# ivargr/kmer_mapper

Hardware: AMD Instinct MI355X
Metric: M k-mers mapped/sec (whole node), k=31 150bp reads (higher is better)
Workload: dtype u64

## Files before the change

kmer_mapper_amd/csrc/kmm_radix.hpp:

```cpp
#pragma once
#include <type_traits>
#include "kmm_radix_plan.hpp"

constexpr int RX_NT = 512;
constexpr int RX_KPT = RX_B / RX_NT;
#ifndef RX_LPR2V
#define RX_LPR2V 16
#endif
constexpr int RX_LPR = RX_LPR2V;
constexpr int RX_NG = RX_NT / RX_LPR;
#ifndef RX_RB1
#define RX_RB1 4
#endif
#ifndef RX_RB2
#define RX_RB2 8
#endif
constexpr int RX_SUBCAP = 1024;
#ifndef RX_SUBCAP3V
#define RX_SUBCAP3V 3072
#endif
constexpr int RX_SUBCAP3 = RX_SUBCAP3V;
#ifndef RX_LPR3
#define RX_LPR3 16
#endif
// ... 77 lines not shown
    const uint64_t quo = fastdiv_m31(q, (uint32_t)iv.modulo, iv.magic, &h);
    *coarse = h >> sh;
    return (quo << sh) | (uint64_t)(h & ((1u << sh) - 1u));
}

__device__ __forceinline__ uint2 rx_pair(const uint32_t *s_in, int c0, int n)
{
    const uint2 p = *reinterpret_cast<const uint2 *>(s_in + c0);
    return make_uint2(c0 < n ? p.x : 0u, c0 + 1 < n ? p.y : 0u);
}

template <bool ONEBAR>
__device__ __forceinline__ uint32_t rx_scan256(const uint32_t *s_in, uint32_t *s_out, int n, uint32_t *s_wave, const int tid)
{
    if (ONEBAR) {
    (void)s_wave;
    const int lane = tid & 63;
    const int wave = __builtin_amdgcn_readfirstlane(tid >> 6);
    if (wave < 4) {
        const uint32_t v = tid < n ? s_in[tid] : 0u;
        const uint32_t inc = wave_scan_incl(v);
        uint32_t before = 0;
        for (int x = 0; x < wave; ++x) {
            const uint32_t t = x * 64 + lane < n ? s_in[x * 64 + lane] : 0u;
            before += (uint32_t)__builtin_amdgcn_readlane((int)wave_scan_incl(t), 63);
        }
        if (tid < n)
            s_out[tid] = before + inc - v;
        if (tid == 255)
            s_out[n] = before + inc;
    }
    __syncthreads();
    return s_out[n];
    }
    const int lane = tid & 63, wave = tid >> 6;
    const uint32_t v = tid < n ? s_in[tid] : 0u;
    const uint32_t inc = wave_scan_incl(v);
    if (wave < 4 && lane == 63)
        s_wave[wave] = inc;
    __syncthreads();
    const uint32_t total = s_wave[0] + s_wave[1] + s_wave[2] + s_wave[3];
    if (tid < n) {
        uint32_t base = 0;
        for (int x = 0; x < wave; ++x)
            base += s_wave[x];
        s_out[tid] = base + inc - v;
    }
    if (tid == 0)
        s_out[n] = total;
    __syncthreads();
    return total;
}

template <bool ONEBAR>
__device__ __forceinline__ uint32_t rx_scan512(const uint32_t *s_in, uint32_t *s_out, int n, uint32_t *s_wave, const int tid)
{
    const int lane = tid & 63;
    const int wave = __builtin_amdgcn_readfirstlane(tid >> 6);
    if (ONEBAR) {
    (void)s_wave;
    if (wave < 4) {
        const int c0 = wave * 128 + lane * 2;
        const uint2 p = rx_pair(s_in, c0, n);
        const uint32_t v = p.x + p.y;
        const uint32_t inc = wave_scan_incl(v);
        uint32_t before = 0;
        for (int x = 0; x < wave; ++x) {
            const uint2 t = rx_pair(s_in, x * 128 + lane * 2, n);
            before += (uint32_t)__builtin_amdgcn_readlane((int)wave_scan_incl(t.x + t.y), 63);
        }
        const uint32_t ex = before + inc - v;
        if (c0 < n)
            s_out[c0] = ex;
        if (c0 + 1 < n)
            s_out[c0 + 1] = ex + p.x;
        if (tid == 255)
            s_out[n] = before + inc;
    }
    __syncthreads();
    return s_out[n];
    }
    uint2 p = make_uint2(0u, 0u);
    uint32_t v = 0, inc = 0;
    const int c0 = wave * 128 + lane * 2;
    if (wave < 4) {
        p = rx_pair(s_in, c0, n);
        v = p.x + p.y;
        inc = wave_scan_incl(v);
        if (lane == 63)
            s_wave[wave] = inc;
    }
    __syncthreads();
    const uint32_t total = s_wave[0] + s_wave[1] + s_wave[2] + s_wave[3];
    if (wave < 4) {
        uint32_t base = 0;
        for (int x = 0; x < wave; ++x)
            base += s_wave[x];
        const uint32_t ex = base + inc - v;
        if (c0 < n)
            s_out[c0] = ex;
        if (c0 + 1 < n)
            s_out[c0 + 1] = ex + p.x;
    }
    if (tid == 0)
        s_out[n] = total;
    __syncthreads();
    return total;
}

#ifdef RX_PHASE_TIMERS
#define RX_PT_DECL unsigned long long pt_acc[7] = {0, 0, 0, 0, 0, 0, (unsigned long long)clock64()}
#define RX_PT_ARG , pt_acc
#define RX_PT_ARG2 , pt_acc
#define RX_PT(slot)                                                                                                   \
    do {                                                                                                              \
        if (threadIdx.x == 0) {                                                                                       \
            const unsigned long long pt_now = (unsigned long long)clock64();                                                            \
            pt_acc[slot] += pt_now - pt_acc[6];                                                                       \
            pt_acc[6] = pt_now;                                                                                       \
        }                                                                                                             \
    } while (0)
#define RX_PT_END(iv, base)                                                                                           \
    do {                                                                                                              \
        if (threadIdx.x == 0)                                                                                         \
            for (int pt_i = 0; pt_i < 6; ++pt_i)                                                                      \
                atomicAdd(&(iv).stats[(size_t)(blockIdx.x % KMM_STAT_SHARDS) * KMM_STAT_STRIDE + (base) + pt_i],     \
                          pt_acc[pt_i]);                                                                              \
    } while (0)
#else
#define RX_PT_DECL
#define RX_PT_ARG
#define RX_PT_ARG2 , nullptr
#define RX_PT(slot)
#define RX_PT_END(iv, base)
#endif

__device__ __forceinline__ int rx_tid_now(int wave)
{
    int l;
    asm volatile("v_mbcnt_lo_u32_b32 %0, -1, 0\n\tv_mbcnt_hi_u32_b32 %0, -1, %0" : "=v"(l));
    return (wave << 6) | l;
}

__device__ __forceinline__ uint32_t rx_spare_key()
{
    return (uint32_t)RX_MAXF + 1u + (threadIdx.x & 63);
}

struct RxNoHook {
    __device__ __forceinline__ void operator()() const {}
};

template <int RB, bool ENDBAR, bool ONEBAR, int NT = RX_NT, bool NTSTORE = ONEBAR, typename PrepFn,
          typename MidFn = RxNoHook, int WAVESCAN = 0, bool NOWTID = false, typename PostFn = RxNoHook, int CAPMAX = RX_B>
__device__ __forceinline__ void rx_sort_emit(uint64_t (&q)[RX_B / NT], PrepFn prep, int F, uint64_t *sbuf,
                                             uint32_t *s_cnt, uint32_t *s_base, uint32_t *s_wave,
                                             uint64_t *__restrict__ out, uint16_t *__restrict__ dir_row,
                                             unsigned long long *pt_acc = nullptr, MidFn mid = MidFn(),
                                             int n_slots = RX_B / NT, int wave_s = -1, PostFn post = PostFn(),
                                             uint64_t *probe_out = nullptr, int probe_den = 0, uint32_t cap = RX_B,
                                             unsigned long long *multi_stat = nullptr)
{
    static_assert(CAPMAX <= RX_B && CAPMAX % 2 == 0, "rounds start at 16-byte boundaries of the output");
    constexpr bool ROUNDS = CAPMAX < RX_B;
    auto tid_now = [&]() { return NOWTID ? rx_tid_now(wave_s) : (int)threadIdx.x; };
    constexpr int KPT = RX_B / NT;
    int tid = tid_now();
    (void)pt_acc;
    uint32_t cr[KPT];
#pragma unroll
    for (int h = 0; h < KPT; h += RB) {
        if (h >= n_slots) {
#pragma unroll
            for (int i = 0; i < RB; ++i)
                cr[h + i] = 0xFFFF0000u;
            continue;
        }
        uint32_t ck[RB], rk[RB];
#pragma unroll
        for (int i = 0; i < RB; ++i)
            ck[i] = prep(h + i);
#pragma unroll
        for (int i = 0; i < RB; ++i)
            rk[i] = atomicAdd(&s_cnt[ck[i]], 1u);
#pragma unroll
        for (int i = 0; i < RB; ++i)
            cr[h + i] = (ck[i] << 16) | (rk[i] & 0xFFFFu);
    }
    __syncthreads();
    RX_PT(2);
    mid();
    uint32_t total;
    uint32_t packed = 0;
    const bool by_wave = WAVESCAN == 2 || (WAVESCAN == 1 && F <= 128);
    auto pos_of = [&](int h) {
        const uint32_t key = cr[h] >> 16;
        if (by_wave) {
            const uint32_t pk = (uint32_t)__builtin_amdgcn_ds_bpermute((int)((key >> 1) << 2), (int)packed);
            return (pk & 0xFFFFu) + ((key & 1u) ? pk >> 16 : 0u) + (cr[h] & 0xFFFFu);
        }
        return s_base[key < (uint32_t)F ? key : 0u] + (cr[h] & 0xFFFFu);
    };
    auto place_first = [&]() {
#pragma unroll
        for (int h = 0; h < KPT; ++h) {
            if (h >= n_slots)
                break;
            const uint32_t pos = pos_of(h);
            if ((cr[h] >> 16) < (uint32_t)F && pos < cap)
                sbuf[pos] = q[h];
        }
    };
    if (by_wave) {
        const int lane = tid & 63;
        const uint2 p = rx_pair(s_cnt, lane * 2, F);
        const uint32_t inc = wave_scan_incl(p.x + p.y);
        const uint32_t ex0 = inc - p.x - p.y;
        total = (uint32_t)__builtin_amdgcn_readlane((int)inc, 63);
        if (tid < 64) {
            if (2 * lane <= F)
                dir_row[2 * lane] = (uint16_t)ex0;
            if (2 * lane + 1 <= F)
                dir_row[2 * lane + 1] = (uint16_t)(ex0 + p.x);
            if (lane == 63 && F == 128)
                dir_row[128] = (uint16_t)inc;
        }
        packed = ex0 | (p.x << 16);
        if (ROUNDS && total > cap) {
            place_first();
        } else {
#pragma unroll
        for (int h = 0; h < KPT; ++h) {
            if (h >= n_slots)
                break;
            const uint32_t key = cr[h] >> 16;
            const uint32_t pk = (uint32_t)__builtin_amdgcn_ds_bpermute((int)((key >> 1) << 2), (int)packed);
            const uint32_t pos = (pk & 0xFFFFu) + ((key & 1u) ? pk >> 16 : 0u) + (cr[h] & 0xFFFFu);
            if (key < (uint32_t)F)
                sbuf[pos] = q[h];
        }
        }
    } else {
    tid = tid_now();
    total = F <= 256 ? rx_scan256<ONEBAR>(s_cnt, s_base, F, s_wave, tid) : rx_scan512<ONEBAR>(s_cnt, s_base, F, s_wave, tid);
    tid = tid_now();
    if (tid <= F)
        s_cnt[tid] = 0;
    if (NT == RX_MAXF && F == NT && tid == 0)
        s_cnt[NT] = 0;
    if (tid <= F)
        dir_row[tid] = (uint16_t)s_base[tid];
    if (NT == RX_MAXF && F == NT && tid == 0)
        dir_row[NT] = (uint16_t)s_base[NT];
    if (ROUNDS && total > cap) {
        place_first();
    } else {
#pragma unroll
    for (int h = 0; h < KPT; ++h) {
        if (h >= n_slots)
            break;
        const uint32_t pos = s_base[cr[h] >> 16] + (cr[h] & 0xFFFFu);
        if ((cr[h] >> 16) < (uint32_t)F)
            sbuf[pos] = q[h];
    }
    }
    }
    post();
    __syncthreads();
    RX_PT(3);
    tid = tid_now();
    if (by_wave) {
        if (tid <= F)
            s_cnt[tid] = 0;
        if (NT == RX_MAXF && F == NT && tid == 0)
            s_cnt[NT] = 0;
    }
    const uint4 *s4 = reinterpret_cast<const uint4 *>(sbuf);
    uint4 *o4 = reinterpret_cast<uint4 *>(out);
    const uint32_t n_first = ROUNDS && total > cap ? cap : total;
    for (uint32_t i = tid; i < (n_first + 1) / 2; i += NT) {
        if (NTSTORE) {
            typedef uint32_t u32x4_t __attribute__((ext_vector_type(4)));
            const uint4 v = s4[i];
            const u32x4_t w = {v.x, v.y, v.z, v.w};
            __builtin_nontemporal_store(w, reinterpret_cast<u32x4_t *>(o4) + i);
        } else {
            o4[i] = s4[i];
        }
        if (RX_PROBE_ANY && probe_den > 0 && i % (uint32_t)probe_den == 0u) {
            if (NTSTORE) {
                typedef uint32_t u32x4_t __attribute__((ext_vector_type(4)));
                const uint4 v = s4[i];
                const u32x4_t w = {v.x, v.y, v.z, v.w};
                __builtin_nontemporal_store(w, reinterpret_cast<u32x4_t *>(probe_out) + i / (uint32_t)probe_den);
            } else {
                reinterpret_cast<uint4 *>(probe_out)[i / (uint32_t)probe_den] = s4[i];
            }
        }
    }
    if constexpr (ROUNDS) {
        if (total > cap) {
            for (uint32_t lo = cap; lo < total; lo += cap) {
                __syncthreads();
#pragma unroll
                for (int h = 0; h < KPT; ++h) {
                    if (h >= n_slots)
                        break;
                    const uint32_t pos = pos_of(h) - lo;
                    if ((cr[h] >> 16) < (uint32_t)F && pos < cap)
                        sbuf[pos] = q[h];
                }
                __syncthreads();
                const uint32_t n = total - lo < cap ? total - lo : cap;
                uint4 *o4r = reinterpret_cast<uint4 *>(out + lo);
                for (uint32_t i = tid; i < (n + 1) / 2; i += NT)
                    o4r[i] = s4[i];
            }
            if (multi_stat && tid == 0)
                atomicAdd(multi_stat, 1ull);
        }
    }
    if (ENDBAR)
        __syncthreads();
    RX_PT(4);
}

__device__ __forceinline__ void rx_stat_add(const IndexView &iv, int which, uint32_t v)
{
#pragma unroll
    for (int d = 32; d > 0; d >>= 1)
        v += __shfl_xor(v, d);
    if ((threadIdx.x & 63) == 0 && v)
        atomicAdd(&iv.stats[(size_t)((blockIdx.x * 8 + (threadIdx.x >> 6)) % KMM_STAT_SHARDS) * KMM_STAT_STRIDE + which],
                  (unsigned long long)v);
}

__device__ __forceinline__ uint32_t rx_scan_threads(uint32_t v, uint32_t (*s_wave8)[RX_NT / 64], uint32_t &flip,
                                                    uint32_t *total)
{
    const int lane = threadIdx.x & 63, wave = threadIdx.x >> 6;
    const uint32_t inc = wave_scan_incl(v);
    uint32_t *row = s_wave8[flip];
    flip ^= 1u;
    if (lane == 63)
        row[wave] = inc;
    __syncthreads();
    uint32_t base = 0, tot = 0;
#pragma unroll
    for (int x = 0; x < RX_NT / 64; ++x) {
        const uint32_t t = row[x];
        base += x < wave ? t : 0u;
        tot += t;
    }
    *total = tot;
    return base + inc - v;
}

template <int LPR, bool LINECUT>
__device__ __forceinline__ uint32_t rx_n_pieces(uint32_t len, uint64_t src)
{
    const uint32_t off = LINECUT ? (uint32_t)src & (uint32_t)(LPR - 1) : 0u;
    return len ? (off + len + LPR - 1) / LPR : 0u;
}

template <int LPR, bool LINECUT>
__device__ __forceinline__ void rx_list_subruns(uint32_t pre, uint32_t len, uint64_t src, uint32_t dst, uint32_t win,
                                                uint32_t *sub_src, uint32_t *sub_meta)
{
    const uint32_t off = LINECUT ? (uint32_t)src & (uint32_t)(LPR - 1) : 0u;
    const uint32_t nsub = rx_n_pieces<LPR, LINECUT>(len, src);
    const uint32_t j0 = pre > win ? pre : win;
    const uint32_t j1 = pre + nsub < win + (uint32_t)RX_SUBCAP ? pre + nsub : win + (uint32_t)RX_SUBCAP;
    for (uint32_t j = j0; j < j1; ++j) {
        const uint32_t p = j - pre;
        const uint32_t a = p ? 0u : off;
        const uint32_t done = p ? p * LPR - off : 0u;
        const uint32_t n = len - done < (uint32_t)LPR - a ? len - done : (uint32_t)LPR - a;
        sub_src[j - win] = (uint32_t)(src - off) + p * LPR;
        sub_meta[j - win] = ((dst + done) << 12) | (a << 6) | n;
    }
}

template <int STEP>
__device__ __forceinline__ void rx_pad_list(uint32_t n, uint32_t *sub_src, uint32_t *sub_meta)
{
    static_assert(RX_SUBCAP % STEP == 0, "a padded list must fit the window");
    const uint32_t n_pad = (n + STEP - 1) / STEP * STEP;
    for (uint32_t i = n + threadIdx.x; i < n_pad; i += RX_NT) {
        sub_src[i] = 0u;
        sub_meta[i] = 0u;
    }
}

__device__ __forceinline__ uint32_t rx_xcc_id()
{
    return (uint32_t)__builtin_amdgcn_s_getreg((3 << 11) | 20) & 7u;
}

__device__ __forceinline__ uint32_t rx_pop(unsigned long long *counters, uint32_t sub, uint32_t limit)
{
    const unsigned long long u = atomicAdd(&counters[sub * 16], 1ull);
    return u < (unsigned long long)limit ? (uint32_t)u : limit;
}

template <int MODE, bool RC, bool C2 = false>
__global__ void __launch_bounds__(RX_NT, 4) k_rx_p1(ReadsView rv, const uint64_t *__restrict__ kmers_in, int64_t n_in,
                                                 IndexView iv, RxView rx, int k, int64_t tile_begin, uint32_t n_src)
{
    constexpr bool PACKED = MODE == MODE_PACKED;
#ifndef RX_P1_STAGE_EARLY
#define RX_P1_STAGE_EARLY 1
#endif
    constexpr bool STAGE_EARLY = PACKED && !RC && RX_P1_STAGE_EARLY != 0;
    constexpr int TM = (MODE == MODE_KMERS || PACKED) ? MODE_UNIFORM : MODE;
    constexpr int S = TM == MODE_RECORDS ? 4 : 16;
    constexpr int R = RX_KPT / S;
    using Smem = typename std::conditional<PACKED, TilePackedSmem, TileSmem<S>>::type;
    using Raw = typename std::conditional<PACKED, TilePackedRaw, TileRaw>::type;
    __shared__ Smem sm[2];
    __shared__ uint64_t sbuf[RX_B];
    __shared__ __attribute__((aligned(8))) uint32_t s_cnt[RX_MAXF + 2 + 64];
    __shared__ uint32_t s_base[RX_MAXF + 1], s_wave[4];
#ifndef RX_P1_INCDIV
#define RX_P1_INCDIV 1
#endif
    constexpr bool INCDIV = RX_P1_INCDIV != 0 && !RC && MODE == MODE_PACKED;
    __shared__ uint4 s_qr[4];
    const int tid = threadIdx.x, half = tid >> 8, ltid = tid & 255;
    const int wave_s = __builtin_amdgcn_readfirstlane(tid >> 6);
    if (INCDIV && tid < 4) {
        uint32_t r;
        const uint64_t qc = fastdiv_m31((uint64_t)tid << (2 * (k - 1)), (uint32_t)iv.modulo, iv.magic, &r);
        s_qr[tid] = make_uint4(r, (uint32_t)qc, (uint32_t)(qc >> 32), 0u);
    }
    TileConst tc;
    tc.kmask = 0; tc.bmask = 0; tc.aligned = false;
    if (MODE != MODE_KMERS) {
        sm[half].lut[ltid] = rv.lut[ltid];
        tc = tile_const(rv, k);
    }
    constexpr uint32_t X = RC ? 2u : 1u;
    const int F1 = (int)rx.F1;
    uint32_t lookups = 0;
    const int sh = rx.w + rx.f2;
    const uint32_t spare = rx_spare_key();
    RX_PT_DECL;
#ifndef RX_P1_NO_PREFETCH
    constexpr bool PREFETCH = R == 1 && MODE != MODE_KMERS;
#else
    constexpr bool PREFETCH = false;
#endif
    Raw pw[R];
    if (tid <= F1)
        s_cnt[tid] = 0;
    if (tid == 0)
        s_cnt[RX_NT] = 0;
    __syncthreads();
    auto load_tile = [&](int64_t tile, Raw &raw) {
        if constexpr (PACKED)
            tile_packed_load<C2>(rv, tile, ltid, raw);
        else
            tile_load_vec<S, TM, C2>(rv, tc, tile, ltid, raw);
    };
#ifndef RX_P1_CHUNKED
#define RX_P1_CHUNKED 0
#endif
    const uint32_t sb_per = (n_src + gridDim.x - 1) / gridDim.x;
    const uint32_t sb_first = RX_P1_CHUNKED ? blockIdx.x * sb_per : blockIdx.x;
    const uint32_t sb_end = RX_P1_CHUNKED ? (sb_first + sb_per < n_src ? sb_first + sb_per : n_src) : n_src;
    const uint32_t sb_step = RX_P1_CHUNKED ? 1u : gridDim.x;
    for (uint32_t sb = sb_first; sb < sb_end; sb += sb_step) {
        uint64_t q[RX_KPT];
        uint32_t valid = 0;
        TileWin win;
        win.lo = win.hi = 0;
        if (MODE == MODE_KMERS) {
#pragma unroll
            for (int i = 0; i < RX_KPT; ++i) {
                const int64_t idx = (int64_t)sb * RX_B + i * RX_NT + tid;
                q[i] = 0;
                if (idx < n_in) {
                    q[i] = __builtin_nontemporal_load(&kmers_in[idx]);
                    valid |= 1u << i;
                }
            }
        } else {
            if constexpr (STAGE_EARLY) {
                const int64_t tile = tile_begin + ((int64_t)sb * 2 + half);
                if (sb == sb_first) {
                    load_tile(tile, pw[0]);
                    tile_packed_stage<C2>(rv, tile, sm[half], ltid, pw[0]);
                    __syncthreads();
                }
                valid = tile_packed_fetch(rv, tc, tile, sm[half], q, ltid, &win);
                if (sb + sb_step < sb_end)
                    load_tile(tile_begin + ((int64_t)(sb + sb_step) * 2 + half), pw[0]);
            } else {
            if (!PREFETCH || sb == sb_first) {
#pragma unroll
                for (int r = 0; r < R; ++r)
                    load_tile(tile_begin + ((int64_t)sb * 2 + half) * R + r, pw[r]);
            }
#pragma unroll
            for (int r = 0; r < R; ++r) {
                uint64_t qq[S];
                const int64_t tile = tile_begin + ((int64_t)sb * 2 + half) * R + r;
                uint32_t v;
                if constexpr (PACKED)
                    v = tile_packed_kmers<false, C2>(rv, tc, tile, k, sm[half], qq, ltid, pw[r], &win);
                else
                    v = r == 0 ? tile_kmers<S, TM, false, C2>(rv, tc, tile, k, sm[half], qq, ltid, pw[r], &win)
                               : tile_kmers<S, TM, true, C2>(rv, tc, tile, k, sm[half], qq, ltid, pw[r]);
#pragma unroll
                for (int j = 0; j < S; ++j)
                    q[r * S + j] = qq[j];
                valid |= v << (r * S);
            }
            if (PREFETCH && sb + sb_step < sb_end) {
#pragma unroll
                for (int r = 0; r < R; ++r)
                    load_tile(tile_begin + ((int64_t)(sb + sb_step) * 2 + half) * R + r, pw[r]);
            }
            }
        }
        lookups += (uint32_t)__popc(valid) * X;
        RX_PT(0);
        if (RC) {
            uint64_t x[RX_KPT];
            auto fwd = [&](int i) {
                uint32_t c;
                x[i] = rx_pack(iv, sh, q[i], &c);
                return ((valid >> i) & 1u) ? c : spare;
            };
            rx_sort_emit<RX_RB1, true, true, RX_NT, true, decltype(fwd), RxNoHook, 0, true>(
                x, fwd, F1, sbuf, s_cnt, s_base, s_wave, rx.buf1 + (size_t)sb * 2 * RX_B,
                rx.start1 + (size_t)sb * 2 * (size_t)(F1 + 1) RX_PT_ARG2, RxNoHook(), RX_KPT, wave_s);
            auto rev = [&](int i) {
                uint32_t c;
                x[i] = rx_pack(iv, sh, revcomp(q[i], k), &c);
                return ((valid >> i) & 1u) ? c : spare;
            };
            rx_sort_emit<RX_RB1, MODE == MODE_KMERS, true, RX_NT, true, decltype(rev), RxNoHook, 0, true>(
                x, rev, F1, sbuf, s_cnt, s_base, s_wave, rx.buf1 + ((size_t)sb * 2 + 1) * RX_B,
                rx.start1 + ((size_t)sb * 2 + 1) * (size_t)(F1 + 1) RX_PT_ARG2, RxNoHook(), RX_KPT, wave_s);
        } else {
            uint32_t qlo = 0, qhi = 0, rem = 0;
            const uint32_t M32 = (uint32_t)iv.modulo, Ml = M32 & 0xFFFFu, Mh = M32 >> 16;
            const uint32_t nb = (uint32_t)((win.lo >> (2 * k)) | (win.hi << (64 - 2 * k)));
            uint4 e_nx = make_uint4(0u, 0u, 0u, 0u);
            auto fwd = [&](int i) {
                if constexpr (INCDIV && R == 1) {
                    const uint4 e = e_nx;
                    if (i + 1 < RX_KPT) {
                        uint32_t c = (nb >> (2 * i)) & 3u;
                        asm("" : "+v"(c) : "v"(rem));
                        e_nx = s_qr[c];
                    }
                    if (i == 0) {
                        const uint64_t quot = fastdiv_m31(win.lo & tc.kmask, M32, iv.magic, &rem);
                        qlo = (uint32_t)quot;
                        qhi = (uint32_t)(quot >> 32);
                    } else {
                        const uint32_t t = qlo & 3u;
                        uint32_t th = __umul24(t, Mh);
                        asm("" : "+v"(th));
                        const uint32_t y = ((__umul24(t, Ml) + rem) >> 2) + (th << 14);
                        const uint32_t r2 = y + e.x;
                        uint32_t nlo, nhi;
                        asm("v_alignbit_b32 %0, %3, %2, 2\n\t"
                            "v_lshrrev_b32 %1, 2, %3\n\t"
                            "v_cmp_le_u32 vcc, %6, %7\n\t"
                            "v_addc_co_u32 %0, vcc, %0, %4, vcc\n\t"
                            "v_addc_co_u32 %1, vcc, %1, %5, vcc"
                            : "=&v"(nlo), "=&v"(nhi)
                            : "v"(qlo), "v"(qhi), "v"(e.y), "v"(e.z), "s"(M32), "v"(r2)
                            : "vcc");
                        qlo = nlo;
                        qhi = nhi;
                        rem = r2 - M32 < r2 ? r2 - M32 : r2;
                    }
                    q[i] = ((((uint64_t)qhi << 32) | qlo) << sh) | (uint64_t)(rem & ((1u << sh) - 1u));
                    return ((valid >> i) & 1u) ? rem >> sh : spare;
                } else {
                    uint32_t c;
                    q[i] = rx_pack(iv, sh, q[i], &c);
                    return ((valid >> i) & 1u) ? c : spare;
                }
            };
            auto post = [&]() {
                if constexpr (STAGE_EARLY) {
                    if (sb + sb_step < sb_end)
                        tile_packed_stage<C2>(rv, tile_begin + ((int64_t)(sb + sb_step) * 2 + half), sm[half], ltid, pw[0]);
                }
            };
            rx_sort_emit<RX_RB1, MODE == MODE_KMERS, true, RX_NT, true, decltype(fwd), RxNoHook, 0, true, decltype(post)>(
                q, fwd, F1, sbuf, s_cnt, s_base, s_wave, rx.buf1 + (size_t)sb * RX_B,
                rx.start1 + (size_t)sb * (size_t)(F1 + 1) RX_PT_ARG2, RxNoHook(), RX_KPT, wave_s, post,
                RX_PROBE_P1W ? rx.probe + (size_t)sb * RX_B : nullptr, RX_PROBE_P1W);
        }
    }
#ifdef RX_PT_P1
    RX_PT_END(iv, 10);
#endif
    rx_stat_add(iv, 0, lookups);
    rx_stat_add(iv, KMM_STAT_RX_P1, lookups);
}

__global__ void __launch_bounds__(256) k_rx_colsum(RxView rx)
{
    const uint32_t F1 = rx.F1;
    const uint32_t b0 = blockIdx.x * RX_CH;
    const uint32_t b1 = b0 + RX_CH < rx.NB ? b0 + RX_CH : rx.NB;
    const size_t ld = F1 + 1;
    for (uint32_t c = threadIdx.x; c < F1; c += 256) {
        const uint16_t *p = rx.start1 + (size_t)b0 * ld + c;
        uint32_t sum = 0, b = b0;
        for (; b + 8 <= b1; b += 8, p += 8 * ld) {
            uint32_t lo[8], hi[8];
#pragma unroll
            for (int u = 0; u < 8; ++u) {
                lo[u] = p[u * ld];
                hi[u] = p[u * ld + 1];
            }
#pragma unroll
            for (int u = 0; u < 8; ++u)
                sum += hi[u] - lo[u];
        }
        for (; b < b1; ++b, p += ld)
            sum += (uint32_t)p[1] - (uint32_t)p[0];
        rx.csum[(size_t)blockIdx.x * F1 + c] = sum;
    }
}

__device__ __forceinline__ uint32_t scan256_excl(uint32_t v, uint32_t *s_wave4, uint32_t *total)
{
    const int lane = threadIdx.x & 63, wave = threadIdx.x >> 6;
    const uint32_t inc = wave_scan_incl(v);
    __syncthreads();
    if (lane == 63)
        s_wave4[wave] = inc;
    __syncthreads();
    uint32_t base = 0;
    for (int x = 0; x < wave; ++x)
        base += s_wave4[x];
    *total = s_wave4[0] + s_wave4[1] + s_wave4[2] + s_wave4[3];
    return base + inc - v;
}

template <bool WITH_P>
__global__ void __launch_bounds__(256) k_rx_chunkscan(RxView rx, uint32_t n_chunks)
{
    __shared__ uint32_t s_wave4[4];
    const uint32_t c = blockIdx.x, F1 = rx.F1;
    uint32_t carry = 0;
    for (uint32_t base = 0; base < n_chunks; base += 256) {
        const uint32_t ch = base + threadIdx.x;
        const uint32_t v = ch < n_chunks ? rx.csum[(size_t)ch * F1 + c] : 0u;
        uint32_t tot;
        const uint32_t ex = scan256_excl(v, s_wave4, &tot);
        if (ch < n_chunks)
            rx.csum[(size_t)ch * F1 + c] = carry + ex;
        carry += tot;
    }
    if (threadIdx.x == 0) {
        rx.T1[c] = carry;
        if constexpr (WITH_P)
            rx.P1T[(size_t)c * (rx.NB + 1) + rx.NB] = carry;
    }
}

__device__ __forceinline__ uint32_t scan512_excl(uint32_t v, uint32_t *s_wave8, uint32_t *total)
{
    const int lane = threadIdx.x & 63, wave = threadIdx.x >> 6;
    const uint32_t inc = wave_scan_incl(v);
    __syncthreads();
    if (lane == 63)
        s_wave8[wave] = inc;
    __syncthreads();
    uint32_t base = 0, tot = 0;
    for (int x = 0; x < 8; ++x) {
        base += x < wave ? s_wave8[x] : 0u;
        tot += s_wave8[x];
    }
    *total = tot;
    return base + inc - v;
}

__global__ void __launch_bounds__(512) k_rx_tables(RxView rx)
{
    static_assert(RX_MAXF <= 512, "one thread per coarse partition");
    __shared__ uint32_t s_wave8[8];
    const uint32_t c = threadIdx.x, F1 = rx.F1;
    const uint32_t run = c < F1 ? rx.T1[c] : 0u;
    const uint32_t n_items = c < F1 ? (run + RX_B - 1) / RX_B : 0u;
    const uint32_t rows = (n_items + RX_IC - 1) / RX_IC;
    uint32_t tot_items, tot_rows;
    const uint32_t ib = scan512_excl(n_items, s_wave8, &tot_items);
    const uint32_t wb = scan512_excl(rows, s_wave8, &tot_rows);
    uint32_t jmax = n_items;
#pragma unroll
    for (int d = 32; d > 0; d >>= 1) {
        const uint32_t o = __shfl_xor(jmax, d);
        jmax = o > jmax ? o : jmax;
    }
    __syncthreads();
    if ((threadIdx.x & 63) == 0)
        s_wave8[threadIdx.x >> 6] = jmax;
    __syncthreads();
    if (c < F1) {
        rx.item_base[c] = ib;
        rx.work_base[c] = wb;
    }
    if (c == 0) {
        uint32_t m = s_wave8[0];
        for (int x = 1; x < 8; ++x)
            m = s_wave8[x] > m ? s_wave8[x] : m;
        rx.item_base[F1] = tot_items;
        rx.work_base[F1] = tot_rows;
        rx.ctrl[0] = tot_items;
        rx.ctrl[1] = tot_rows;
        rx.ctrl[2] = m;
    }
}

template <bool WITH_P>
__global__ void __launch_bounds__(256) k_rx_colscan(RxView rx)
{
    constexpr int RB = 32;
    constexpr int TB = WITH_P ? 32 : 64, CW = 256;
    static_assert(RX_CH % TB == 0 && TB % RB == 0, "a chunk is whole tiles, a tile whole register rounds");
    __shared__ uint32_t tP[WITH_P ? CW : 1][TB + 1];
    __shared__ uint16_t tS[CW][TB + 2];
    const uint32_t F1 = rx.F1, NB = rx.NB;
    const uint32_t b0 = blockIdx.x * RX_CH;
    const uint32_t b1 = b0 + RX_CH < NB ? b0 + RX_CH : NB;
    const size_t ld = F1 + 1;
    const uint32_t lane = threadIdx.x & 63, wave = threadIdx.x >> 6;
    {
    const uint32_t cb = blockIdx.y * CW;
    const uint32_t c = cb + threadIdx.x;
    const uint32_t nc = F1 - cb < (uint32_t)CW ? F1 - cb : (uint32_t)CW;
    uint32_t run = c < F1 ? rx.csum[(size_t)blockIdx.x * F1 + c] : 0u;
    const uint32_t ib = c < F1 ? rx.item_base[c] : 0u;
    for (uint32_t t0 = b0; t0 < b1; t0 += TB) {
        const uint32_t nb = b1 - t0 < (uint32_t)TB ? b1 - t0 : (uint32_t)TB;
        if (c < F1) {
#pragma unroll 1
            for (uint32_t r0 = 0; r0 < (uint32_t)TB; r0 += RB) {
                const uint16_t *p = rx.start1 + (size_t)(t0 + r0) * ld + c;
                uint32_t lo[RB], hi[RB];
#pragma unroll
                for (int u = 0; u < RB; ++u) {
                    lo[u] = r0 + (uint32_t)u < nb ? p[u * ld] : 0u;
                    hi[u] = r0 + (uint32_t)u < nb ? p[u * ld + 1] : 0u;
                }
#pragma unroll
                for (int u = 0; u < RB; ++u) {
                    const uint32_t cnt = hi[u] - lo[u];
                    if constexpr (WITH_P)
                        tP[threadIdx.x][r0 + u] = run;
                    tS[threadIdx.x][r0 + u] = (uint16_t)lo[u];
                    if (cnt) {
                        uint32_t m = (run + RX_B - 1) / RX_B;
                        while ((uint64_t)m * RX_B < (uint64_t)run + cnt) {
                            rx.item_desc[ib + m] = make_uint2(t0 + r0 + u, WITH_P ? c : run);
                            ++m;
                        }
                    }
                    run += cnt;
                }
            }
        }
        __syncthreads();
        if constexpr (WITH_P) {
            const uint32_t bi = lane & 31;
            for (uint32_t cc = wave * 2 + (lane >> 5); cc < nc; cc += 8) {
                if (bi < nb) {
                    rx.P1T[(size_t)(cb + cc) * (NB + 1) + t0 + bi] = tP[cc][bi];
                    rx.S1T[(size_t)(cb + cc) * NB + t0 + bi] = tS[cc][bi];
                }
            }
        } else {
            for (uint32_t cc = wave; cc < nc; cc += 4) {
                if (lane < nb)
// ... 1186 lines not shown
```

kmer_mapper_amd/csrc/kmm_radix_host.hpp:

```cpp
#pragma once

int rx_check_conservation(kmm_index *ix)
{
    if (!ix->rx_unchecked)
        return KMM_OK;
    ix->rx_unchecked = false;
    static thread_local std::vector<unsigned long long> st;
    st.resize(KMM_STAT_BYTES / 8);
    HIPCHK(hipMemcpy(st.data(), ix->stats, KMM_STAT_BYTES, hipMemcpyDeviceToHost));
    unsigned long long p1 = 0, p2 = 0, p3 = 0, dropped = 0;
    for (int i = 0; i < KMM_STAT_SHARDS; ++i) {
        const unsigned long long *sh = st.data() + (size_t)i * KMM_STAT_STRIDE;
        p1 += sh[KMM_STAT_RX_P1];
        p2 += sh[2];
        p3 += sh[3];
        dropped += sh[KMM_STAT_RX_DROPPED];
    }
    if (p1 == p2 && p2 == p3 + dropped)
        return KMM_OK;
    const int rc = fail(KMM_ERR_INTERNAL, "radix path self-check failed: pass 1 emitted %llu k-mers, pass 2 gathered %llu, "
                        "pass 3 probed %llu (+ %llu dropped as absent) since the counters were last reset: the node counts "
                        "are invalid until kmm_reset_counts [latest map call #%llu on this handle]",
                        p1, p2, p3, dropped, (unsigned long long)ix->map_calls);
    ix->sticky_rc = rc;
// ... 30 lines not shown
    return ix->rx_p3_fp && rx_p3_shape(rx_p3_variant(ix)).fingerprints;
}

RxView rx_view_of(const kmm_index *ix, const RxScratch &sc, uint32_t NB)
{
    const RxGeometry &g = ix->rx_geo;
    RxView rx;
    memset(&rx, 0, sizeof rx);
    rx.pstart = ix->rx_pstart; rx.pkeys = ix->rx_pkeys; rx.pfreq = ix->rx_pfreq; rx.ecnt = ix->rx_ecnt;
    rx.pstart16 = ix->rx_pstart16; rx.slice_e0 = ix->rx_slice_e0; rx.slice_fmax = ix->rx_slice_fmax;
    rx.occ = ix->rx_occ;
    rx.slots = rx_slots_active(ix) ? (const uint32_t *)ix->rx_slots : nullptr;
    rx.p2f_cap = ix->dbg_p2f_cap;
    rx.occ_shift = rx_filter_active(ix) ? g.occ_shift : 3;
    rx.p2f_k = NB / 2048u < 4u ? 4u : (NB / 2048u > (uint32_t)P2F_KMAX ? (uint32_t)P2F_KMAX : NB / 2048u);
    rx.w = g.w; rx.f2 = g.f2; rx.PF = g.PF; rx.F1 = g.F1; rx.F2 = g.F2;
    rx.NB = NB; rx.max_items = (uint32_t)sc.max_items;
    uint8_t *m = (uint8_t *)ix->rx_meta.p;
    rx.start1 = (uint16_t *)(m + sc.start1); rx.P1T = (uint32_t *)(m + sc.P1T); rx.S1T = (uint16_t *)(m + sc.S1T);
    rx.csum = (uint32_t *)(m + sc.csum); rx.T1 = (uint32_t *)(m + sc.T1); rx.item_base = (uint32_t *)(m + sc.item_base);
    rx.work_base = (uint32_t *)(m + sc.work_base); rx.item_desc = (uint2 *)(m + sc.item_desc);
    rx.start2 = (uint16_t *)(m + sc.start2); rx.start2T = (uint16_t *)(m + sc.start2T);
    rx.ctrl = (uint32_t *)(m + sc.ctrl);
    rx.queue = (unsigned long long *)(m + sc.queue);
    rx.buf1 = (uint64_t *)ix->rx_buf1.p;
    rx.buf2 = (uint64_t *)ix->rx_buf2.p;
#if RX_PROBE_ANY
    rx.probe = (uint64_t *)ix->rx_probe.p;
#endif
    return rx;
}

template <int MODE>
int rx_launch_p1(kmm_index *ix, const ReadsView &rv, const uint64_t *src_kmers, int64_t n_kmers, const IndexView &iv,
                 const RxView &rx, int k, int64_t tile0, uint32_t n_src, int also_rc)
{
    static const int p1_per_cu = getenv("KMM_RX_P1_GRID_PER_CU") ? atoi(getenv("KMM_RX_P1_GRID_PER_CU")) : 8;
    const int64_t g1cap = (int64_t)ix->n_cu * (p1_per_cu > 0 ? p1_per_cu : 8);
    const dim3 g1((unsigned)(n_src < g1cap ? n_src : g1cap));
    constexpr bool CAN_C2 = MODE == MODE_PACKED || MODE == MODE_UNIFORM || MODE == MODE_GENERAL;
    if (rv.codes2 && !CAN_C2)
        return fail(KMM_ERR_INTERNAL, "2-bit code input reaches pass 1 through the flat-read modes only");
    auto go = [&](auto kern) {
        hipLaunchKernelGGL(kern, g1, dim3(RX_NT), 0, ix->stream, rv, src_kmers, n_kmers, iv, rx, k, tile0, n_src);
    };
    if constexpr (CAN_C2) {
        if (rv.codes2) {
            if (also_rc)
                go(k_rx_p1<MODE, true, true>);
            else
                go(k_rx_p1<MODE, false, true>);
            return KMM_OK;
        }
    }
    if (also_rc)
        go(k_rx_p1<MODE, true>);
    else
        go(k_rx_p1<MODE, false>);
    return KMM_OK;
}

void rx_launch_p2(kmm_index *ix, const IndexView &iv, const RxView &rx)
{
    if (!ix->rx_filter) {
        hipLaunchKernelGGL(k_rx_p2, dim3(ix->n_cu * ix->rx_grid_per_cu), dim3(RX_NT), 0, ix->stream, iv, rx);
        return;
    }
    const bool flt = rx_filter_active(ix), small = rx.F2 <= 128;
    auto kern = rx.slots ? (small ? k_rx_p2f<P2F_SLOT, true> : k_rx_p2f<P2F_SLOT, false>)
                : flt    ? (small ? k_rx_p2f<P2F_BITMAP, true> : k_rx_p2f<P2F_BITMAP, false>)
                         : (small ? k_rx_p2f<P2F_NONE, true> : k_rx_p2f<P2F_NONE, false>);
    hipLaunchKernelGGL(kern, dim3(ix->n_cu), dim3(P2F_NT), 0, ix->stream, iv, rx);
}

void rx_launch_p3(kmm_index *ix, const IndexView &iv, const RxView &rx, int max_freq)
{
    const RxP3Variant v = rx_p3_variant(ix);
    const dim3 grid(ix->n_cu * (rx_p3_shape(v).wg_per_cu > 1 ? ix->rx_grid_per_cu : 1));
    auto go = [&](auto kern) { hipLaunchKernelGGL(kern, grid, dim3(RX_NT), 0, ix->stream, iv, rx, max_freq); };
    static_assert(rx_p3_shape(RxP3Variant::W12_DIR16).fingerprints && rx_p3_fp_shapes() == 1,
                  "RX_P3_SHAPES promises the fingerprint form exactly where an instantiation is named below");
    switch (v) {
    case RxP3Variant::W12_DIR16:
        if (rx_p3_fp_active(ix))
            go(k_rx_p3<RX_WMAX, RX_ECAP, 4, uint16_t, RX_SUBCAP3, true, true>);
        else
            go(k_rx_p3<RX_WMAX, RX_ECAP, 4, uint16_t, RX_SUBCAP3, true>);
        break;
    case RxP3Variant::W12:             go(k_rx_p3<RX_WMAX, RX_ECAP, 4, uint32_t>); break;
    case RxP3Variant::W13_SMALL_DIR16: go(k_rx_p3<RX_WMAX_BIG, RX_ECAP, 4, uint16_t, RX_SUBCAP3, true>); break;
    case RxP3Variant::W13_SMALL:       go(k_rx_p3<RX_WMAX_BIG, RX_ECAP, 4, uint16_t>); break;
    case RxP3Variant::W13_MID_DIR16:   go(k_rx_p3<RX_WMAX_BIG, RX_ECAP_MID, 4, uint16_t, 1024, true>); break;
    case RxP3Variant::W13_MID:         go(k_rx_p3<RX_WMAX_BIG, RX_ECAP_MID, 4, uint16_t, 1024>); break;
    case RxP3Variant::W13_BIG:         go(k_rx_p3<RX_WMAX_BIG, RX_ECAP_BIG, 2, uint32_t>); break;
    }
}

template <int MODE>
int launch_rx(kmm_index *ix, const ReadsView &rv, const uint64_t *kmers_in, int64_t n_in, int k, int max_freq,
              int also_rc)
{
    const IndexView iv = view_of(ix);
    const int64_t units = MODE == MODE_KMERS ? n_in : rv.total;
    const int64_t n_src_total = MODE == MODE_PACKED ? (rv.n_reads + 2 * (int64_t)rv.pk_rpt - 1) / (2 * (int64_t)rv.pk_rpt)
                                                    : (units + RX_B - 1) / RX_B;
    const uint32_t X = also_rc ? 2u : 1u;
    const uint32_t F1 = ix->rx_geo.F1, F2 = ix->rx_geo.F2;
    RxSplit split;
    static const bool verbose = getenv("KMM_VERBOSE") != nullptr;
    const auto t_0 = std::chrono::steady_clock::now();
    if (ix->rx_sub_cap_eff > 0 && ++ix->rx_sub_cap_eff_age >= RX_SUB_CAP_AGE)
        ix->rx_sub_cap_eff = 0;
    int64_t cap = ix->rx_sub_cap_eff > 0 && ix->rx_sub_cap_eff < ix->rx_sub_cap ? ix->rx_sub_cap_eff : ix->rx_sub_cap;
    for (;;) {
        split = rx_split(n_src_total, X, cap);
        const RxScratch sm = rx_scratch((uint32_t)(split.max_src * X), F1, F2);
        int rc = ix->dbg_rx_buf_limit && sm.buf1_bytes > (size_t)ix->dbg_rx_buf_limit ? (int)KMM_ERR_NOMEM
                                                                                      : ensure(ix->rx_meta, sm.meta_bytes);
        if (rc == KMM_OK)
            rc = ensure(ix->rx_buf1, sm.buf1_bytes);
        if (rc == KMM_OK)
            rc = ensure(ix->rx_buf2, sm.buf2_bytes);
#if RX_PROBE_ANY
        if (rc == KMM_OK)
            rc = ensure(ix->rx_probe, sm.buf2_bytes);
#endif
        if (rc == KMM_OK)
            break;
        if (rc != KMM_ERR_NOMEM || cap <= RX_SUB_CAP_FLOOR || n_src_total <= 1)
            return rc;
        (void)hipGetLastError();
        (void)ix->rx_buf1.reset();
        (void)ix->rx_buf2.reset();
        cap = rx_next_smaller_cap(n_src_total, X, split.n_sub);
        ix->rx_sub_cap_eff = cap;
        ix->rx_sub_cap_eff_age = 0;
    }
    ix->rx_sub_cap_last = cap;
    const double ms_buffers = ms_since(t_0);
    const int64_t max_src = split.max_src;
    for (int64_t s0 = 0; s0 < n_src_total; s0 += max_src) {
        const uint32_t n_src = (uint32_t)(n_src_total - s0 < max_src ? n_src_total - s0 : max_src);
        const uint32_t NB = n_src * X;
        const RxScratch sc = rx_scratch(NB, F1, F2);
        bool grew = sc.meta_bytes > ix->rx_meta.cap || sc.buf1_bytes > ix->rx_buf1.cap || sc.buf2_bytes > ix->rx_buf2.cap;
#if RX_PROBE_ANY
        grew = grew || sc.buf2_bytes > ix->rx_probe.cap;
#endif
        if (grew)
            return fail(KMM_ERR_INTERNAL, "radix path: a sub-batch of %u blocks needs more scratch than the largest one was given", NB);
        const RxView rx = rx_view_of(ix, sc, NB);
        ix->dbg_T1 = rx.T1; ix->dbg_item_base = rx.item_base; ix->dbg_start1 = rx.start1; ix->dbg_F1 = F1; ix->dbg_NB = NB;
        HIPCHK(hipMemsetAsync(rx.ctrl, 0, sc.meta_bytes - sc.ctrl, ix->stream));
        ScopedTimer tm;
        KMMCHK(tm.begin(ix, KMM_KERNEL_RX_P1));
        const int64_t tile0 = s0 * (RX_B / (MODE == MODE_RECORDS ? 1024 : 4096));
        KMMCHK(rx_launch_p1<MODE>(ix, rv, kmers_in ? kmers_in + s0 * RX_B : nullptr, n_in - s0 * RX_B, iv, rx, k, tile0, n_src,
                                  also_rc));
        HIPCHK(hipGetLastError());
        KMMCHK(tm.end());
        KMMCHK(tm.begin(ix, KMM_KERNEL_RX_SCAN));
        const bool with_p = !ix->rx_filter;
        auto chunkscan = with_p ? k_rx_chunkscan<true> : k_rx_chunkscan<false>;
        auto colscan = with_p ? k_rx_colscan<true> : k_rx_colscan<false>;
        hipLaunchKernelGGL(k_rx_colsum, dim3(sc.chunks), dim3(256), 0, ix->stream, rx);
        hipLaunchKernelGGL(chunkscan, dim3(F1), dim3(256), 0, ix->stream, rx, sc.chunks);
        hipLaunchKernelGGL(k_rx_tables, dim3(1), dim3(512), 0, ix->stream, rx);
        hipLaunchKernelGGL(colscan, dim3(sc.chunks, (F1 + 255) / 256), dim3(256), 0, ix->stream, rx);
        HIPCHK(hipGetLastError());
        KMMCHK(tm.end());
        KMMCHK(tm.begin(ix, KMM_KERNEL_RX_P2));
        rx_launch_p2(ix, iv, rx);
        HIPCHK(hipGetLastError());
        KMMCHK(tm.end());
        KMMCHK(tm.begin(ix, KMM_KERNEL_RX_SCAN));
        hipLaunchKernelGGL(k_rx_tr2, dim3((unsigned)((sc.max_items + RX_TR2 - 1) / RX_TR2)), dim3(256), 0, ix->stream, rx);
        HIPCHK(hipGetLastError());
        KMMCHK(tm.end());
        KMMCHK(tm.begin(ix, KMM_KERNEL_RX_P3));
        rx_launch_p3(ix, iv, rx, max_freq);
        HIPCHK(hipGetLastError());
        KMMCHK(tm.end());
        ix->ecnt_dirty = true;
        ix->rx_unchecked = true;
    }
    ix->n_radix_batches++;
    if (verbose && ms_since(t_0) > 20.0)
        fprintf(stderr, "libkmm: radix passes of %lld positions: %.2f ms for the batch buffers (%zu + %zu + %zu bytes), %.2f ms to issue %lld "
                "sub-batch(es)\n", (long long)units, ms_buffers, ix->rx_meta.cap, ix->rx_buf1.cap, ix->rx_buf2.cap, ms_since(t_0) - ms_buffers,
                (long long)split.n_sub);
    return KMM_OK;
}

int rx_flush(kmm_index *ix)
{
    if (!ix->ecnt_dirty)
        return KMM_OK;
    ScopedTimer tm;
    KMMCHK(tm.begin(ix, KMM_KERNEL_RX_FLUSH));
    if (ix->rx_norder && !ix->rx_ecnt_acc && ix->rx_flush_sorted) {
        hipLaunchKernelGGL(k_rx_flush_sorted, dim3(ix->n_cu * 8), dim3(256), 0, ix->stream, view_of(ix), ix->rx_ecnt,
                           ix->rx_norder, ix->rx_nnode, ix->rx_S);
        HIPCHK(hipMemsetAsync(ix->rx_ecnt, 0, (size_t)ix->rx_S * 4, ix->stream));
    } else {
        hipLaunchKernelGGL(k_rx_flush, dim3(ix->n_cu * 8), dim3(256), 0, ix->stream, view_of(ix), ix->rx_ecnt,
                           ix->rx_pnodes, ix->rx_S, ix->rx_ecnt_acc);
    }
    HIPCHK(hipGetLastError());
    KMMCHK(tm.end());
    ix->ecnt_dirty = false;
    return KMM_OK;
}

int rx_build_slots(kmm_index *ix)
{
    static_cast<RxSlotFilter &>(*ix) = RxSlotFilter();
    if (!ix->rx_filter || !ix->rx_geo.slot_filter || !ix->rx_filter_slots || !ix->rx_occ)
        return KMM_OK;
    const size_t bytes = (size_t)ix->rx_geo.F1 * P2F_SLOT_WORDS * 4;
    if (hipMalloc(ix->rx_slots.put(), bytes) != hipSuccess) {
        (void)hipGetLastError();
        static_cast<RxSlotFilter &>(*ix) = RxSlotFilter();
        return KMM_OK;
    }
    HIPCHK(hipMemsetAsync(ix->rx_slots, 0, bytes, ix->stream));
    hipLaunchKernelGGL(k_rx_build_slots, dim3(grid_for(ix, (int64_t)((ix->modulo + 255) / 256), 16)), dim3(256), 0, ix->stream,
                       ix->rx_pstart, ix->rx_pkeys, ix->modulo, ix->rx_geo.w + ix->rx_geo.f2, ix->rx_slots);
    HIPCHK(hipGetLastError());
    HIPCHK(hipStreamSynchronize(ix->stream));
    return KMM_OK;
}

int rx_repack_keys(kmm_index *ix)
{
    if (ix->rx_S)
        hipLaunchKernelGGL(k_rx_pack_keys, dim3(grid_for(ix, (int64_t)((ix->rx_S + 255) / 256), 16)), dim3(256), 0,
                           ix->stream, ix->rx_pkeys_raw, ix->rx_S, view_of(ix), ix->rx_geo.w + ix->rx_geo.f2, ix->rx_pkeys);
    HIPCHK(hipGetLastError());
    HIPCHK(hipMemsetAsync(ix->queue, 0, 3 * sizeof(unsigned long long), ix->stream));
    hipLaunchKernelGGL(k_rx_max_slice, dim3(grid_for(ix, (int64_t)((ix->rx_geo.PF + 255) / 256), 16)), dim3(256), 0, ix->stream,
                       ix->rx_pstart, ix->modulo, ix->rx_geo.w, ix->rx_geo.PF, ix->queue);
    HIPCHK(hipGetLastError());
    unsigned long long mx[3] = {0, 0, 0};
    HIPCHK(hipMemcpyAsync(mx, ix->queue, sizeof mx, hipMemcpyDeviceToHost, ix->stream));
    HIPCHK(hipStreamSynchronize(ix->stream));
    ix->rx_max_slice = (uint32_t)mx[0];
    const unsigned long long odd = ix->rx_geo.PF / 1000 > 1 ? ix->rx_geo.PF / 1000 : 1;
    ix->rx_fits_small = mx[1] <= odd;
    ix->rx_fits_mid = mx[2] <= odd;
    static_cast<RxDir16 &>(*ix) = RxDir16();
    if (ix->rx_max_slice <= 65535u && !getenv("KMM_RX_NO_P16")) {
        const size_t n16 = ((size_t)ix->rx_geo.PF << ix->rx_geo.w) + 8;
        if (hipMalloc(ix->rx_pstart16.put(), n16 * 2) == hipSuccess &&
            hipMalloc(ix->rx_slice_e0.put(), ((size_t)ix->rx_geo.PF + 2) * 4) == hipSuccess &&
            hipMalloc(ix->rx_slice_fmax.put(), ((size_t)ix->rx_geo.PF + 2) * 2) == hipSuccess) {
            hipLaunchKernelGGL(k_rx_pstart16, dim3(grid_for(ix, (int64_t)((n16 + 255) / 256), 16)), dim3(256), 0, ix->stream,
                               ix->rx_pstart, ix->modulo, ix->rx_geo.w, ix->rx_geo.PF, ix->rx_pstart16, ix->rx_slice_e0);
            HIPCHK(hipGetLastError());
            hipLaunchKernelGGL(k_rx_slice_fmax, dim3(grid_for(ix, (int64_t)((ix->rx_geo.PF + 3) / 4), 16)), dim3(256), 0, ix->stream,
                               ix->rx_slice_e0, ix->rx_pfreq, ix->rx_geo.PF, ix->rx_slice_fmax);
            HIPCHK(hipGetLastError());
            HIPCHK(hipStreamSynchronize(ix->stream));
        } else {
            (void)hipGetLastError();
            static_cast<RxDir16 &>(*ix) = RxDir16();
        }
    }
    return rx_build_slots(ix);
}

int rx_build(kmm_index *ix, const int32_t *h2i, const int32_t *nk, const uint64_t *kmers, const int32_t *nodes,
             const uint16_t *freqs)
{
    const uint64_t M = ix->modulo;
    if (const char *env = getenv("KMM_RX_FILTER"))
        ix->rx_filter = atoi(env) != 0;
    if (const char *env = getenv("KMM_RX_FILTER_SLOTS"))
        ix->rx_filter_slots = atoi(env) != 0;
    if (const char *env = getenv("KMM_RX_P3_FP"))
        ix->rx_p3_fp = atoi(env) != 0;
    ix->rx_why_not = 1;
    if (M >= (1ull << 31))
        return KMM_OK;
    DevBuf sizes;
    std::vector<DevBuf> scratch(2 * SCAN_MAX_LEVELS);
    int rc = KMM_OK;
    hipError_t e = hipSuccess;
    bool overlap = false;
    do {
        if ((rc = ensure(sizes, (size_t)(M + 1) * 4))) break;
        if ((e = hipMalloc(ix->rx_pstart.put(), (size_t)(M + 1) * RxViewBytes::pstart))) break;
        hipLaunchKernelGGL(k_rx_bucket_sizes, dim3(grid_for(ix, (int64_t)((M + 256) / 256), 16)), dim3(256), 0,
                           ix->stream, h2i, nk, M, ix->n_entries, (uint32_t *)sizes.p);
        unsigned long long sum64 = 0;
        if ((e = hipMemsetAsync(ix->queue, 0, sizeof(unsigned long long), ix->stream))) break;
        hipLaunchKernelGGL(k_sum_u32, dim3(grid_for(ix, (int64_t)((M + 256) / 256), 8)), dim3(256), 0, ix->stream,
                           (const uint32_t *)sizes.p, M + 1, ix->queue);
        if ((e = hipMemcpyAsync(&sum64, ix->queue, 8, hipMemcpyDeviceToHost, ix->stream))) break;
        if ((e = hipStreamSynchronize(ix->stream))) break;
        if (sum64 > (unsigned long long)ix->n_entries) {
            overlap = true;
            break;
        }
        if ((rc = scan_exclusive((const uint32_t *)sizes.p, ix->rx_pstart, M + 1, scratch, 0, ix->stream))) break;
        uint32_t total = 0;
        if ((e = hipMemcpyAsync(&total, ix->rx_pstart + M, 4, hipMemcpyDeviceToHost, ix->stream))) break;
        if ((e = hipStreamSynchronize(ix->stream))) break;
        ix->rx_S = total;
        {
            const size_t occ_words = (size_t)((M + 31) / 32) + ((size_t)1 << (P2F_LOGBITS + 2 - 5));
            if (hipMalloc(ix->rx_occ.put(), occ_words * 4) == hipSuccess) {
                if ((e = hipMemsetAsync(ix->rx_occ, 0, occ_words * 4, ix->stream))) break;
                hipLaunchKernelGGL(k_rx_build_occ, dim3(grid_for(ix, (int64_t)((M / 32 + 256) / 256), 16)), dim3(256), 0, ix->stream,
                                   ix->rx_pstart, M, ix->rx_occ);
            } else {
                (void)hipGetLastError();
            }
        }
// ... 96 lines not shown
```

Before: 177,500.

## Fuse per-chunk bucket column sums into radix pass 1 via shared accumulators

Pass 1 now accumulates per-bucket counts in a shared-memory array while it clears them after each block scan. At each chunk boundary it flushes the counts to the global chunk-sum table with atomic adds. This removes the separate colsum kernel, which re-read the whole start1 directory. To keep each block's work inside contiguous chunks, the grid-stride loop over sub-batches becomes a contiguous balanced split. The cost is an extra memset, extra shared memory and atomics, plus the change in access pattern and load balance from contiguous assignment.

```diff
diff --git a/kmer_mapper_amd/csrc/kmm_radix.hpp b/kmer_mapper_amd/csrc/kmm_radix.hpp
--- a/kmer_mapper_amd/csrc/kmm_radix.hpp
+++ b/kmer_mapper_amd/csrc/kmm_radix.hpp
@@ -253,16 +253,18 @@
 };
 
 template <int RB, bool ENDBAR, bool ONEBAR, int NT = RX_NT, bool NTSTORE = ONEBAR, typename PrepFn,
-          typename MidFn = RxNoHook, int WAVESCAN = 0, bool NOWTID = false, typename PostFn = RxNoHook, int CAPMAX = RX_B>
+          typename MidFn = RxNoHook, int WAVESCAN = 0, bool NOWTID = false, typename PostFn = RxNoHook, int CAPMAX = RX_B,
+          bool COLSUM = false>
 __device__ __forceinline__ void rx_sort_emit(uint64_t (&q)[RX_B / NT], PrepFn prep, int F, uint64_t *sbuf,
                                              uint32_t *s_cnt, uint32_t *s_base, uint32_t *s_wave,
                                              uint64_t *__restrict__ out, uint16_t *__restrict__ dir_row,
                                              unsigned long long *pt_acc = nullptr, MidFn mid = MidFn(),
                                              int n_slots = RX_B / NT, int wave_s = -1, PostFn post = PostFn(),
                                              uint64_t *probe_out = nullptr, int probe_den = 0, uint32_t cap = RX_B,
-                                             unsigned long long *multi_stat = nullptr)
+                                             unsigned long long *multi_stat = nullptr, uint32_t *col_acc = nullptr)
 {
     static_assert(CAPMAX <= RX_B && CAPMAX % 2 == 0, "rounds start at 16-byte boundaries of the output");
+    static_assert(!COLSUM || (WAVESCAN == 0 && CAPMAX == RX_B), "the counts are taken where the workgroup scan clears them");
     constexpr bool ROUNDS = CAPMAX < RX_B;
     auto tid_now = [&]() { return NOWTID ? rx_tid_now(wave_s) : (int)threadIdx.x; };
     constexpr int KPT = RX_B / NT;
@@ -345,8 +347,11 @@
     tid = tid_now();
     total = F <= 256 ? rx_scan256<ONEBAR>(s_cnt, s_base, F, s_wave, tid) : rx_scan512<ONEBAR>(s_cnt, s_base, F, s_wave, tid);
     tid = tid_now();
-    if (tid <= F)
+    if (tid <= F) {
+        if constexpr (COLSUM)
+            col_acc[tid] += s_cnt[tid];
         s_cnt[tid] = 0;
+    }
     if (NT == RX_MAXF && F == NT && tid == 0)
         s_cnt[NT] = 0;
     if (tid <= F)
@@ -522,6 +527,7 @@
     __shared__ uint64_t sbuf[RX_B];
     __shared__ __attribute__((aligned(8))) uint32_t s_cnt[RX_MAXF + 2 + 64];
     __shared__ uint32_t s_base[RX_MAXF + 1], s_wave[4];
+    __shared__ uint32_t s_col[RX_MAXF + 1];
 #ifndef RX_P1_INCDIV
 #define RX_P1_INCDIV 1
 #endif
@@ -552,8 +558,10 @@
     constexpr bool PREFETCH = false;
 #endif
     Raw pw[R];
-    if (tid <= F1)
+    if (tid <= F1) {
         s_cnt[tid] = 0;
+        s_col[tid] = 0;
+    }
     if (tid == 0)
         s_cnt[RX_NT] = 0;
     __syncthreads();
@@ -563,13 +571,11 @@
         else
             tile_load_vec<S, TM, C2>(rv, tc, tile, ltid, raw);
     };
-#ifndef RX_P1_CHUNKED
-#define RX_P1_CHUNKED 0
-#endif
-    const uint32_t sb_per = (n_src + gridDim.x - 1) / gridDim.x;
-    const uint32_t sb_first = RX_P1_CHUNKED ? blockIdx.x * sb_per : blockIdx.x;
-    const uint32_t sb_end = RX_P1_CHUNKED ? (sb_first + sb_per < n_src ? sb_first + sb_per : n_src) : n_src;
-    const uint32_t sb_step = RX_P1_CHUNKED ? 1u : gridDim.x;
+    static_assert(RX_CH % 2 == 0, "the two rows of a block (RC) lie in one chunk");
+    const uint32_t sb_q = n_src / gridDim.x, sb_r = n_src % gridDim.x;
+    const uint32_t sb_first = blockIdx.x * sb_q + (blockIdx.x < sb_r ? blockIdx.x : sb_r);
+    const uint32_t sb_end = sb_first + sb_q + (blockIdx.x < sb_r ? 1u : 0u);
+    constexpr uint32_t sb_step = 1u;
     for (uint32_t sb = sb_first; sb < sb_end; sb += sb_step) {
         uint64_t q[RX_KPT];
         uint32_t valid = 0;
@@ -633,17 +639,19 @@
                 x[i] = rx_pack(iv, sh, q[i], &c);
                 return ((valid >> i) & 1u) ? c : spare;
             };
-            rx_sort_emit<RX_RB1, true, true, RX_NT, true, decltype(fwd), RxNoHook, 0, true>(
+            rx_sort_emit<RX_RB1, true, true, RX_NT, true, decltype(fwd), RxNoHook, 0, true, RxNoHook, RX_B, true>(
                 x, fwd, F1, sbuf, s_cnt, s_base, s_wave, rx.buf1 + (size_t)sb * 2 * RX_B,
-                rx.start1 + (size_t)sb * 2 * (size_t)(F1 + 1) RX_PT_ARG2, RxNoHook(), RX_KPT, wave_s);
+                rx.start1 + (size_t)sb * 2 * (size_t)(F1 + 1) RX_PT_ARG2, RxNoHook(), RX_KPT, wave_s, RxNoHook(), nullptr, 0,
+                RX_B, nullptr, s_col);
             auto rev = [&](int i) {
                 uint32_t c;
                 x[i] = rx_pack(iv, sh, revcomp(q[i], k), &c);
                 return ((valid >> i) & 1u) ? c : spare;
             };
-            rx_sort_emit<RX_RB1, MODE == MODE_KMERS, true, RX_NT, true, decltype(rev), RxNoHook, 0, true>(
+            rx_sort_emit<RX_RB1, MODE == MODE_KMERS, true, RX_NT, true, decltype(rev), RxNoHook, 0, true, RxNoHook, RX_B, true>(
                 x, rev, F1, sbuf, s_cnt, s_base, s_wave, rx.buf1 + ((size_t)sb * 2 + 1) * RX_B,
-                rx.start1 + ((size_t)sb * 2 + 1) * (size_t)(F1 + 1) RX_PT_ARG2, RxNoHook(), RX_KPT, wave_s);
+                rx.start1 + ((size_t)sb * 2 + 1) * (size_t)(F1 + 1) RX_PT_ARG2, RxNoHook(), RX_KPT, wave_s, RxNoHook(), nullptr, 0,
+                RX_B, nullptr, s_col);
         } else {
             uint32_t qlo = 0, qhi = 0, rem = 0;
             const uint32_t M32 = (uint32_t)iv.modulo, Ml = M32 & 0xFFFFu, Mh = M32 >> 16;
@@ -694,10 +702,19 @@
                         tile_packed_stage<C2>(rv, tile_begin + ((int64_t)(sb + sb_step) * 2 + half), sm[half], ltid, pw[0]);
                 }
             };
-            rx_sort_emit<RX_RB1, MODE == MODE_KMERS, true, RX_NT, true, decltype(fwd), RxNoHook, 0, true, decltype(post)>(
+            rx_sort_emit<RX_RB1, MODE == MODE_KMERS, true, RX_NT, true, decltype(fwd), RxNoHook, 0, true, decltype(post), RX_B, true>(
                 q, fwd, F1, sbuf, s_cnt, s_base, s_wave, rx.buf1 + (size_t)sb * RX_B,
                 rx.start1 + (size_t)sb * (size_t)(F1 + 1) RX_PT_ARG2, RxNoHook(), RX_KPT, wave_s, post,
-                RX_PROBE_P1W ? rx.probe + (size_t)sb * RX_B : nullptr, RX_PROBE_P1W);
+                RX_PROBE_P1W ? rx.probe + (size_t)sb * RX_B : nullptr, RX_PROBE_P1W, RX_B, nullptr, s_col);
+        }
+        if (((sb + 1u) * X) % (uint32_t)RX_CH == 0u || sb + 1u == sb_end) {
+            const int t = rx_tid_now(wave_s);
+            if (t < F1) {
+                const uint32_t v = s_col[t];
+                s_col[t] = 0;
+                if (v)
+                    atomicAdd(&rx.csum[(size_t)((sb * X) / (uint32_t)RX_CH) * (size_t)F1 + t], v);
+            }
         }
     }
 #ifdef RX_PT_P1
@@ -705,32 +722,6 @@
 #endif
     rx_stat_add(iv, 0, lookups);
     rx_stat_add(iv, KMM_STAT_RX_P1, lookups);
-}
-
-__global__ void __launch_bounds__(256) k_rx_colsum(RxView rx)
-{
-    const uint32_t F1 = rx.F1;
-    const uint32_t b0 = blockIdx.x * RX_CH;
-    const uint32_t b1 = b0 + RX_CH < rx.NB ? b0 + RX_CH : rx.NB;
-    const size_t ld = F1 + 1;
-    for (uint32_t c = threadIdx.x; c < F1; c += 256) {
-        const uint16_t *p = rx.start1 + (size_t)b0 * ld + c;
-        uint32_t sum = 0, b = b0;
-        for (; b + 8 <= b1; b += 8, p += 8 * ld) {
-            uint32_t lo[8], hi[8];
-#pragma unroll
-            for (int u = 0; u < 8; ++u) {
-                lo[u] = p[u * ld];
-                hi[u] = p[u * ld + 1];
-            }
-#pragma unroll
-            for (int u = 0; u < 8; ++u)
-                sum += hi[u] - lo[u];
-        }
-        for (; b < b1; ++b, p += ld)
-            sum += (uint32_t)p[1] - (uint32_t)p[0];
-        rx.csum[(size_t)blockIdx.x * F1 + c] = sum;
-    }
 }
 
 __device__ __forceinline__ uint32_t scan256_excl(uint32_t v, uint32_t *s_wave4, uint32_t *total)
diff --git a/kmer_mapper_amd/csrc/kmm_radix_host.hpp b/kmer_mapper_amd/csrc/kmm_radix_host.hpp
--- a/kmer_mapper_amd/csrc/kmm_radix_host.hpp
+++ b/kmer_mapper_amd/csrc/kmm_radix_host.hpp
@@ -206,6 +206,7 @@
         const RxView rx = rx_view_of(ix, sc, NB);
         ix->dbg_T1 = rx.T1; ix->dbg_item_base = rx.item_base; ix->dbg_start1 = rx.start1; ix->dbg_F1 = F1; ix->dbg_NB = NB;
         HIPCHK(hipMemsetAsync(rx.ctrl, 0, sc.meta_bytes - sc.ctrl, ix->stream));
+        HIPCHK(hipMemsetAsync(rx.csum, 0, (size_t)sc.chunks * F1 * 4, ix->stream));
         ScopedTimer tm;
         KMMCHK(tm.begin(ix, KMM_KERNEL_RX_P1));
         const int64_t tile0 = s0 * (RX_B / (MODE == MODE_RECORDS ? 1024 : 4096));
@@ -217,7 +218,6 @@
         const bool with_p = !ix->rx_filter;
         auto chunkscan = with_p ? k_rx_chunkscan<true> : k_rx_chunkscan<false>;
         auto colscan = with_p ? k_rx_colscan<true> : k_rx_colscan<false>;
-        hipLaunchKernelGGL(k_rx_colsum, dim3(sc.chunks), dim3(256), 0, ix->stream, rx);
         hipLaunchKernelGGL(chunkscan, dim3(F1), dim3(256), 0, ix->stream, rx, sc.chunks);
         hipLaunchKernelGGL(k_rx_tables, dim3(1), dim3(512), 0, ix->stream, rx);
         hipLaunchKernelGGL(colscan, dim3(sc.chunks, (F1 + 255) / 256), dim3(256), 0, ix->stream, rx);
```

Result: no change. 178,100 (median of 6 runs) (+0.3%).
